# VasylVaskivskyi/microaligner

Measured on AMD Instinct MI355X. Metric: Mpix/s optical-flow reg+warp, 16k×16k float32 tile, 1/2/4/8 GPU, higher is better.
Workload: dtype f32

## Files before the change

### include/microaligner_hip.h

```cpp
#ifndef MICROALIGNER_HIP_H
#define MICROALIGNER_HIP_H

#include <stddef.h>
#include <stdint.h>

#ifdef __cplusplus
extern "C" {
#endif

typedef struct ma_ctx ma_ctx;

enum ma_dtype { MA_U8 = 0, MA_U16 = 1, MA_F32 = 2 };

enum ma_status {
    MA_OK = 0,
    MA_EINVAL = -1,
    MA_ENOMEM = -2,
    MA_EHIP = -3,
    MA_ENODEV = -4
};

enum ma_farneback_flags {
    MA_FB_MULADD_FUSED = 1
};

enum ma_dog_flags {
    MA_DOG_FUSED_BLUR = 1,
    MA_DOG_FUSED_SCALE = 2,
    MA_DOG_REPORT_ASYNC = 4
};

const char* ma_version(void);
const char* ma_last_error(void);
int ma_device_count(int* count);
int ma_ctx_create(int device, ma_ctx** out);
void ma_ctx_destroy(ma_ctx* ctx);
int ma_sync(ma_ctx* ctx);
int ma_ctx_set_workspace_limit(ma_ctx* ctx, size_t bytes);
void* ma_ctx_stream(ma_ctx* ctx);
int ma_ctx_trim(ma_ctx* ctx);
int ma_ctx_transfer_stats(ma_ctx* ctx, unsigned long long* h2d_bytes, unsigned long long* d2h_bytes, int reset);

enum ma_option { MA_OPT_COMPANION_STREAM = 1, MA_OPT_WORKSPACE_LIMIT = 2, MA_OPT_WARP_BAND_BYTES = 3 };
int ma_ctx_set_option(ma_ctx* ctx, int option, long long value);
int ma_ctx_get_option(ma_ctx* ctx, int option, long long* value);

enum ma_engine { MA_ENGINE_COMPUTE = 0, MA_ENGINE_H2D = 1, MA_ENGINE_D2H = 2 };
int ma_engine_memcpy_h2d(ma_ctx* ctx, int engine, void* dst, const void* src_host, size_t bytes);
int ma_engine_memcpy_d2h(ma_ctx* ctx, int engine, void* dst_host, const void* src, size_t bytes);
int ma_engine_record(ma_ctx* ctx, int engine, void* ev);
int ma_engine_wait(ma_ctx* ctx, int engine, void* ev);
int ma_engine_sync(ma_ctx* ctx, int engine);
int ma_host_parallel_copy(void* dst, const void* src, size_t bytes);
int ma_host_stream_copy(void* dst, const void* src, size_t bytes);
int ma_event_sync(ma_ctx* ctx, void* ev);

int ma_device_info(int device, char* name, size_t name_len, char* pci_bus_id, size_t pci_len, size_t* mem_free,
                   size_t* mem_total, int* compute_units);
int ma_clock_probe(ma_ctx* ctx, double milliseconds, double* sustained_ghz);

int ma_malloc(ma_ctx* ctx, size_t bytes, void** dptr);
int ma_free(ma_ctx* ctx, void* dptr);
int ma_memcpy_h2d(ma_ctx* ctx, void* dst, const void* src_host, size_t bytes);
int ma_memcpy_d2h(ma_ctx* ctx, void* dst_host, const void* src, size_t bytes);
int ma_memcpy_d2d(ma_ctx* ctx, void* dst, const void* src, size_t bytes);
int ma_memcpy_d2h_async(ma_ctx* ctx, void* dst_host, const void* src, size_t bytes);
int ma_host_alloc(size_t bytes, void** hptr);
int ma_host_free(void* hptr);
// ... 150 lines not shown
```

### microaligner_amd/_lib.py

```python
import ctypes as C
import os

_HERE = os.path.dirname(os.path.abspath(__file__))
LIB_PATH = os.environ.get("MICROALIGNER_HIP_LIB") or os.path.join(_HERE, "libmicroaligner_hip.so")

MA_U8, MA_U16, MA_F32 = 0, 1, 2
MA_OK, MA_EINVAL, MA_ENOMEM, MA_EHIP, MA_ENODEV = 0, -1, -2, -3, -4
MA_FB_MULADD_FUSED = 1
MA_KNN_AUTO, MA_KNN_EXACT, MA_KNN_FILTERED, MA_KNN_FILTERED_F32 = 0, 1, 2, 3
MA_DOG_FUSED_BLUR, MA_DOG_FUSED_SCALE, MA_DOG_REPORT_ASYNC = 1, 2, 4
MA_FLOW_CELL_REPLICAS = 8
MA_OPT_COMPANION_STREAM, MA_OPT_WORKSPACE_LIMIT, MA_OPT_WARP_BAND_BYTES = 1, 2, 3
MA_ENGINE_COMPUTE, MA_ENGINE_H2D, MA_ENGINE_D2H = 0, 1, 2

KERNEL_IDS = {"polyexp_m0": 0, "blur_v": 1, "blur_h_solve": 2, "warp": 3, "merge": 4, "pyr_down": 5,
              "pyr_up": 6, "dog": 7, "nmi": 8, "other": 9, "fb_level_img": 10, "fb_polyexp_plain": 11,
              "fb_flow_resize": 12, "fb_update_matrices": 13}

_vp, _i, _sz, _d, _f = C.c_void_p, C.c_int, C.c_size_t, C.c_double, C.c_float

SIGNATURES = {
    "ma_version": (C.c_char_p, []),
    "ma_last_error": (C.c_char_p, []),
    "ma_device_count": (_i, [C.POINTER(_i)]),
    "ma_ctx_create": (_i, [_i, C.POINTER(_vp)]),
    "ma_ctx_destroy": (None, [_vp]),
    "ma_sync": (_i, [_vp]),
    "ma_ctx_set_workspace_limit": (_i, [_vp, _sz]),
    "ma_ctx_stream": (_vp, [_vp]),
    "ma_malloc": (_i, [_vp, _sz, C.POINTER(_vp)]),
    "ma_free": (_i, [_vp, _vp]),
    "ma_memcpy_h2d": (_i, [_vp, _vp, _vp, _sz]),
    "ma_memcpy_d2h": (_i, [_vp, _vp, _vp, _sz]),
    "ma_memcpy_d2d": (_i, [_vp, _vp, _vp, _sz]),
    "ma_memcpy_d2h_async": (_i, [_vp, _vp, _vp, _sz]),
# ... 71 lines not shown
                              C.POINTER(MaFeatureRoundResult)]),
    "ma_ctx_trim": (_i, [_vp]),
    "ma_ctx_transfer_stats": (_i, [_vp, C.POINTER(C.c_ulonglong), C.POINTER(C.c_ulonglong), _i]),
    "ma_params_default": (None, [C.POINTER(MaParams)]),
    "ma_optflow_register": (_i, [_vp, _vp, _vp, _i, _i, _i, C.POINTER(MaParams), _vp, C.POINTER(MaLevelReport), _i,
                                 C.POINTER(_i)]),
    "ma_host_np_mean": (_i, [C.POINTER(_d), C.c_long, C.POINTER(_d)]),
    "ma_fast_keypoints": (_i, [_vp, _vp, _i, _i, _i, _i, _i, _vp, C.POINTER(_i)]),
    "ma_cut_tiles_u8": (_i, [_vp, _vp, _i, _i, _i, _i, _i, _i, _vp]),
    "ma_device_info": (_i, [_i, C.c_char_p, _sz, C.c_char_p, _sz, C.POINTER(_sz), C.POINTER(_sz), C.POINTER(_i)]),
    "ma_clock_probe": (_i, [_vp, _d, C.POINTER(_d)]),
    "ma_ctx_set_option": (_i, [_vp, _i, C.c_longlong]),
    "ma_ctx_get_option": (_i, [_vp, _i, C.POINTER(C.c_longlong)]),
    "ma_engine_memcpy_h2d": (_i, [_vp, _i, _vp, _vp, _sz]),
    "ma_engine_memcpy_d2h": (_i, [_vp, _i, _vp, _vp, _sz]),
    "ma_engine_record": (_i, [_vp, _i, _vp]),
    "ma_engine_wait": (_i, [_vp, _i, _vp]),
    "ma_engine_sync": (_i, [_vp, _i]),
    "ma_event_sync": (_i, [_vp, _vp]),
    "ma_host_parallel_copy": (_i, [_vp, _vp, _sz]),
    "ma_host_stream_copy": (_i, [_vp, _vp, _sz]),
    "ma_warp_pages_plan": (_i, [_i, _i, _i, _i, _i, _sz, C.POINTER(_i), C.POINTER(_i)]),
    "ma_convert_f32": (_i, [_vp, _vp, _i, _sz, _vp]),
})

QC_SIGNATURES = {
    "ma_qc_nmi_grid": (_i, [_vp, _vp, _vp, _vp, _i, _i, _i, _i, C.POINTER(_d), C.POINTER(_d), C.POINTER(_d), C.POINTER(_d)]),
    "ma_qc_flow_grid": (_i, [_vp, _vp, _i, _i, _i, _i, C.POINTER(_d), C.POINTER(C.c_longlong), C.POINTER(C.c_longlong),
                             C.POINTER(_d), C.POINTER(_d)]),
}

MA_INTER_NEAREST, MA_INTER_LINEAR, MA_INTER_CUBIC, MA_INTER_LANCZOS4 = 0, 1, 2, 4
INTERP_SIGNATURES = {
    "ma_remap_interp": (_i, [_vp, _vp, _i, _i, _i, _i, _vp, _i, _i, _vp, _i]),
    "ma_warp_tiled_interp": (_i, [_vp, _vp, _i, _i, _i, _vp, _i, _i, _vp, _i]),
    "ma_warp_pages_host_interp": (_i, [_vp, C.POINTER(_vp), C.POINTER(_vp), _i, _i, _i, _i, _vp, _i, _i, _i]),
}

COMPOSE_SIGNATURES = {
    "ma_warp_affine_flow": (_i, [_vp, _vp, _i, _i, _i, _i, _i, _vp, _i, _i, C.POINTER(_d), _vp, _i]),
    "ma_warp_affine_flow_pages_host": (_i, [_vp, C.POINTER(_vp), C.POINTER(_vp), _i, _i, _i, _i, _i, _i, _vp, _i, _i,
                                            C.POINTER(_d), _i]),
}

FLOWCOMPOSE_SIGNATURES = {
    "ma_compose_flows": (_i, [_vp, _vp, _vp, _i, _i, _vp]),
# ... 38 lines not shown
```

### microaligner_amd/csrc/farneback.hip

```cpp
#include "ma_internal.h"

#include <algorithm>
#include <cmath>
#include <cfloat>
#include <type_traits>

namespace {

struct FbGeom {
    MaTiling t;
    int pitch;
    int tile0;
    size_t plane;
    int margin;
};

struct PolyConsts {
    float g0, g1, xg1, xxg1;
    double ig11, ig03, ig33, ig55;
};

enum { PL_R0 = 0, PL_R1 = 5, PL_M = 10, PL_V = 15, PL_COUNT = 20 };

__device__ __forceinline__ float* plane_ptr(float* ws, const FbGeom& g, int wl, int pl)
// ... 204 lines not shown
                for (int k = 0; k < 5; k++)
                    __builtin_amdgcn_raw_buffer_store_b32(__float_as_uint(R[k]), wrsrc, pix4,
                                                          ((img == 0 ? PL_R0 : PL_R1) + k) * plane4, ST_NT);
            }
            if (img == 0) {
#pragma unroll
                for (int k = 0; k < 5; k++) r0v[rr][k] = R[k];
            } else if (ok) {
                const bool inside = x < Pw - 1 && y < Ph - 1;
                float Mv[5];
                update_matrices_px(r0v[rr], R[0], R[1], R[2], R[3], R[4], inside, 0.f, 0.f, x, y, Pw, Ph, Mv);
#pragma unroll
                for (int k = 0; k < 5; k++)
                    __builtin_amdgcn_raw_buffer_store_b32(__float_as_uint(Mv[k]), wrsrc, pix4, (PL_M + k) * plane4, ST_NT);
            }
        }
        __syncthreads();
    }
}

constexpr int BV_WAVES = 6, BH_WAVES = 4;
template <int R, int NW, bool FUSED>
__global__ __launch_bounds__(64 * NW, BV_WAVES) void fb_blur_v(FbGeom g, int m, const float* __restrict__ taps,
                                                     float* __restrict__ ws, int nplanes, int reach)
{
    extern __shared__ float lds[];
    const int lane = threadIdx.x & 63;
    const int w = __builtin_amdgcn_readfirstlane(threadIdx.x >> 6);
    const int Ph = g.t.Ph, Pw = g.t.Pw;
    const int nbx = (Pw + 63) / 64, nby = (Ph + NW * R - 1) / (NW * R);
    const int nslots = (int)(((nplanes + 7) / 8) * 8);
    const int item = d_xcd_work_item(blockIdx.x, nbx * nby * nslots);
    const int by = item % nby, bx = (item / nby) % nbx;
    const int bz = d_xcd_unit(item / (nby * nbx), nplanes);
    if (bz >= nplanes) return;
    const int wl = bz / 5, ch = bz - wl * 5;
    const float* src = plane_ptr(ws, g, wl, PL_M + ch);
    float* dst = plane_ptr(ws, g, wl, PL_V + ch);
    int oy, ox, ey, ex;
    window_origin(g.t, g.tile0 + wl, oy, ox);
    window_extent(g, oy, ox, ey, ex);
    const FbRect need = needed_rect_v(g.t, oy, ox, reach, m);
    const int x0 = (need.x0 & ~(NEED_XALIGN - 1)) + bx * 64, y0 = need.y0 + by * (NW * R);
    if (x0 >= min(ex, need.x1) || y0 >= min(ey, need.y1)) return;

    constexpr int G = 2;
    const int rows = NW * R + 2 * m + 2 * G;
    const int xc = min(x0 + lane, Pw - 1);
    const bool xin = xc < ex;
    {
        constexpr int SB = 42;
        const unsigned xo = (unsigned)xc * 4u;
        const __amdgpu_buffer_rsrc_t rsrc = __builtin_amdgcn_make_buffer_rsrc(const_cast<float*>(src), 0,
                                                                               (int)(g.plane * sizeof(float)), 0x00020000);
        for (int j0 = w; j0 < rows; j0 += NW * SB) {
            float v[SB];
#pragma unroll
            for (int k = 0; k < SB; k++) {
// ... 103 lines not shown
        }
        if (y0 + w * R < yend) {
            int jb = jbase + w * R;
            if (jb >= C) jb -= C;
            float acc[R];
            d_sym_fir_ring_pk<R, FUSED>(lds + lane, jb, C, m, taps, acc);
            if (x >= need.x0 && x < need.x1) {
#pragma unroll
                for (int r = 0; r < R; r++) {
                    const int y = y0 + w * R + r;
                    if (y < need.y1) __builtin_amdgcn_raw_buffer_store_b32(__float_as_uint(acc[r]), drsrc, x * 4, y * g.pitch * 4, 0);
                }
            }
        }
        jbase += CH;
        if (jbase >= C) jbase -= C;
        __syncthreads();
    }
}

template <int R, int NW, bool FUSED, int Q, bool LAST, int ROWS>
__global__ __launch_bounds__(64 * NW, BH_WAVES) void fb_blur_h_solve(FbGeom g, int m, const float* __restrict__ taps,
                                                           float* __restrict__ ws, float* __restrict__ flow_out,
                                                           int nwin, int reach)
{
    extern __shared__ float lds[];
    static_assert(ROWS == 64 || ROWS == 32, "a wave covers 64 rows, or 32 rows twice");
    constexpr int HALVES = 64 / ROWS;
    constexpr int TXW = NW * R * HALVES;
    constexpr int NT = 64 * NW;
    const int tid = threadIdx.x;
    const int lane = tid & 63;
    const int row = lane & (ROWS - 1);
    const int hcol = (lane / ROWS) * (NW * R);
    const int w = __builtin_amdgcn_readfirstlane(tid >> 6);
    const int Ph = g.t.Ph, Pw = g.t.Pw;
    const int nbx = (Pw + TXW - 1) / TXW, nby = (Ph + ROWS - 1) / ROWS;
    const int nslots = (int)(((nwin + 7) / 8) * 8);
    const int item = d_xcd_work_item(blockIdx.x, nbx * nby * nslots);
    const int bx = item % nbx, by = (item / nbx) % nby;
    const int wl = d_xcd_unit(item / (nbx * nby), nwin);
    if (wl >= nwin) return;
    int oy, ox, ey, ex;
    window_origin(g.t, g.tile0 + wl, oy, ox);
    window_extent(g, oy, ox, ey, ex);
    const FbRect need = needed_rect_h(g.t, oy, ox, reach);
    const int x0 = (need.x0 & ~(NEED_XALIGN - 1)) + bx * TXW, y0 = need.y0 + by * ROWS;
    const int xend = min(ex, need.x1), yend = min(ey, need.y1);
    if (x0 >= xend || y0 >= yend) return;
    constexpr int G = 2;
    const int cols = TXW + 2 * m + 2 * G;
    const int lp = cols | 1;

    constexpr int RW = ROWS / NW;
    float v[RW][Q];
    const int plane4 = (int)(g.plane * sizeof(float));
    const __amdgpu_buffer_rsrc_t wrsrc = __builtin_amdgcn_make_buffer_rsrc(plane_ptr(ws, g, wl, 0), 0, PL_COUNT * plane4, 0x00020000);
    int xo[Q];
#pragma unroll
    for (int q = 0; q < Q; q++) {
        const int xi = d_clamp(x0 - m - G + lane + 64 * q, 0, Pw - 1);
        xo[q] = xi >= ex ? (int)0x80000000 : xi * 4;
    }
    auto issue = [&](int ch) {
#pragma unroll
// ... 482 lines not shown
    const size_t lds_t = (size_t)BH_ROWS * (BH_TXW + 1) * 2 * sizeof(float);
    if (lds_t > lds_h) lds_h = lds_t;
    p.fast = m >= 1 && lds_v <= LDS_MAX && lds_h <= LDS_MAX && colsh <= 320;
    g.margin = p.fast ? (iters - 1) * m + 3 : (1 << 28);
    p.px = 0;
    p.px_v.assign(iters, 0.0);
    p.px_h.assign(iters, 0.0);
    for (int wl = 0; wl < nwin; wl++) {
        int oy = 0, ox = 0;
        if (g.t.T > 0) { int ty = (g.tile0 + wl) / g.t.ntx, tx = (g.tile0 + wl) % g.t.ntx; oy = ty * g.t.T - g.t.ov; ox = tx * g.t.T - g.t.ov; }
        const int vy = std::min(Ph, g.t.H - oy), vx = std::min(Pw, g.t.W - ox);
        const int ey = std::min(Ph, vy + std::min(g.margin, Ph)), ex = std::min(Pw, vx + std::min(g.margin, Pw));
        p.px += (double)ey * ex;
        for (int it = 0; it < iters; it++) {
            const int reach = p.fast ? (iters - 1 - it) * m : (1 << 28) / 2;
            const FbRect rh = needed_rect_h(g.t, oy, ox, reach), rv = needed_rect_v(g.t, oy, ox, reach, m);
            p.px_h[it] += (double)std::max(0, std::min(ey, rh.y1) - rh.y0) * std::max(0, std::min(ex, rh.x1) - rh.x0);
            p.px_v[it] += (double)std::max(0, std::min(ey, rv.y1) - rv.y0) * std::max(0, std::min(ex, rv.x1) - rv.x0);
        }
    }
    return p;
}

template <bool FUSED>
void run_iterations(ma_ctx* ctx, const FbGeom& g, const FbPlan& p, int nwin, int m, const float* taps, int iters,
                    float* flow_out)
{
    float* ws = (float*)ctx->ws;
    const int Ph = g.t.Ph, Pw = g.t.Pw;
    const size_t lds_v = (size_t)(BV_NW * BV_R + 2 * m + 4) * 64 * sizeof(float);
    const int colsh = BH_TXW + 2 * m + 4;
    size_t lds_h = (size_t)BH_ROWS * (colsh | 1) * sizeof(float);
    const size_t lds_t = (size_t)BH_ROWS * (BH_TXW + 1) * 2 * sizeof(float);
    if (lds_t > lds_h) lds_h = lds_t;
    const bool fast = p.fast;
    for (int it = 0; it < iters; it++) {
        const int last = it == iters - 1;
        const int reach = (iters - 1 - it) * m;
        if (fast) {
            {
                MaProfScope ps(ctx, MA_K_BLUR_V, p.px_v[it]);
                const size_t lds_vs = (size_t)(BVS_NW * BV_R + 2 * m + 4 + 3 * (BV_R / 2) + 1) * 64 * sizeof(float);
                if (m % (BV_R / 2) == 0 && lds_vs <= LDS_MAX) {
                    const long long items = (long long)((Pw + 63) / 64) * nwin * 5;
                    hipLaunchKernelGGL((fb_blur_v_stream<BV_R, BVS_NW, FUSED>), dim3((unsigned)items), dim3(64 * BVS_NW),
                                       lds_vs, ctx->stream, g, m, taps, ws, nwin * 5, reach);
                } else {
                    const long long items = (long long)((Pw + 63) / 64) * ((Ph + BV_NW * BV_R - 1) / (BV_NW * BV_R)) * ma_xcd_slots(nwin * 5);
                    hipLaunchKernelGGL((fb_blur_v<BV_R, BV_NW, FUSED>), dim3(ma_xcd_grid(items)), dim3(64 * BV_NW), lds_v,
                                       ctx->stream, g, m, taps, ws, nwin * 5, reach);
                }
            }
            {
                MaProfScope ps(ctx, MA_K_BLUR_H_SOLVE, p.px_h[it]);
                const long long items = (long long)((Pw + BH_TXW - 1) / BH_TXW) * ((Ph + BH_ROWS - 1) / BH_ROWS) * ma_xcd_slots(nwin);
#define MA_BLUR_H(QQ)                                                                                               \
    do {                                                                                                            \
        if (last) hipLaunchKernelGGL((fb_blur_h_solve<BH_R, BH_NW, FUSED, QQ, true, BH_ROWS>), dim3(ma_xcd_grid(items)),     \
                                     dim3(64 * BH_NW), lds_h, ctx->stream, g, m, taps, ws, flow_out, nwin, reach);  \
        else hipLaunchKernelGGL((fb_blur_h_solve<BH_R, BH_NW, FUSED, QQ, false, BH_ROWS>), dim3(ma_xcd_grid(items)),         \
                                dim3(64 * BH_NW), lds_h, ctx->stream, g, m, taps, ws, flow_out, nwin, reach);       \
    } while (0)
                if (colsh <= 192) MA_BLUR_H(3);
                else if (colsh <= 256) MA_BLUR_H(4);
                else MA_BLUR_H(5);
#undef MA_BLUR_H
            }
        } else {
            {
                MaProfScope ps(ctx, MA_K_BLUR_V, p.px);
                dim3 grid((Pw + 255) / 256, Ph, nwin * 5);
                hipLaunchKernelGGL((fb_blur_v_simple<FUSED>), grid, dim3(256), 0, ctx->stream, g, m, taps, ws);
            }
            {
                MaProfScope ps(ctx, MA_K_BLUR_H_SOLVE, p.px);
                dim3 grid((Pw + 255) / 256, Ph, nwin);
                hipLaunchKernelGGL((fb_blur_h_solve_simple<FUSED>), grid, dim3(256), 0, ctx->stream, g, m, taps, ws,
                                   last, flow_out);
            }
        }
    }
}

template <typename T, bool FUSED>
int run_batch(ma_ctx* ctx, const T* prev, const T* next, FbGeom g, int nwin, const PolyConsts& pc, int m,
              const float* taps, int iters, float* flow_out)
{
    float* ws = (float*)ctx->ws;
    const FbPlan p = plan_batch(g, nwin, m, iters);
    {
        MaProfScope ps(ctx, MA_K_POLYEXP_M0, p.px);
        dim3 grid((g.t.Pw + K1_TX - 1) / K1_TX, (g.t.Ph + K1_TY - 1) / K1_TY, nwin);
        hipLaunchKernelGGL((fb_polyexp_m0<T>), grid, dim3(K1_THREADS), 0, ctx->stream, prev, next, g, pc, ws);
    }
    run_iterations<FUSED>(ctx, g, p, nwin, m, taps, iters, flow_out);
    MA_HIP(hipGetLastError());
    return MA_OK;
}

int get_taps(ma_ctx* ctx, int winsize, const float** out)
{
    std::vector<float> k;
    make_window_taps(winsize, k);
    std::vector<float> t = ma_layout_taps(k);
    return ma_const_table(ctx, ((uint64_t)1 << 56) | (uint64_t)winsize, t.data(), t.size(), out);
}

int check_window(int Ph, int Pw)
{
    const size_t bytes = ma_fb_window_bytes(Ph, Pw);
    if (bytes <= MA_FB_WINDOW_MAX_BYTES) return MA_OK;
    ma_set_error("invalid argument: Farneback window of %d x %d px too large: its 20 planes take %zu bytes, the 32-bit "
                 "plane addressing allows %zu (5178 x 5178 is the largest square window)", Ph, Pw, bytes,
                 MA_FB_WINDOW_MAX_BYTES);
    return MA_EINVAL;
}

int farneback_impl(ma_ctx* ctx, const void* prev, const void* next, int dtype, int H, int W, int tile, int overlap,
// ... 136 lines not shown
                for (int img = 0; img < 2; img++) {
                    hipLaunchKernelGGL((fb_level_rows<T, FUSED>), dim3((2 * l.w + LV_THREADS - 1) / LV_THREADS,
                                       (unsigned)std::min(H, MA_GRID_Y_MAX)), dim3(LV_THREADS), 0, ctx->stream,
                                       img == 0 ? prev : next, H, W, l.w, sx, dk, l.ksize, tmp);
                    hipLaunchKernelGGL((fb_level_cols<FUSED>), dim3((l.w + 255) / 256, gy), dim3(256), 0, ctx->stream, tmp, H,
                                       W, l.w, l.h, sx, sy, area, dk, l.ksize, ws + (PL_V + img) * g.plane, g.pitch);
                }
            }
            MaProfScope ps(ctx, MA_K_FB_POLYEXP_PLAIN, 2 * px);
            hipLaunchKernelGGL(fb_polyexp_plain, dim3((l.w + 255) / 256, gy, 2), dim3(256), 0, ctx->stream, g, pc, ws);
        }
        if (k == top) {
            MA_HIP(hipMemsetAsync(flow_out, 0, (size_t)l.w * l.h * 2 * sizeof(float), ctx->stream));
        } else {
            const FbLevel& c = L[k + 1];
            MaProfScope ps(ctx, MA_K_FB_FLOW_RESIZE, px);
            hipLaunchKernelGGL((fb_flow_resize<FUSED>), dim3((l.w + 255) / 256, gy), dim3(256), 0, ctx->stream, flow_lv,
                               c.w, c.h, rs_scale(l.w, c.w), rs_scale(l.h, c.h), flow_out, l.w, l.h);
        }
        {
            MaProfScope ps(ctx, MA_K_FB_UPDATE_MATRICES, px);
            hipLaunchKernelGGL(fb_update_matrices, dim3((l.w + 255) / 256, gy), dim3(256), 0, ctx->stream, g, flow_out, ws);
        }
        run_iterations<FUSED>(ctx, g, p, 1, m, taps, iters, k == 0 ? flow_out : flow_lv);
        MA_HIP(hipGetLastError());
    }
    return MA_OK;
}

int farneback_levels_impl(ma_ctx* ctx, const void* prev, const void* next, int dtype, int H, int W, int levels,
                          double pyr_scale, int winsize, int iterations, int poly_n, double poly_sigma, int flags,
                          float* flow_out)
{
    MA_REQUIRE(levels >= 0, "levels must be >= 0");
    MA_REQUIRE(pyr_scale == 0.5, "only pyr_scale == 0.5 is supported");
    if (levels == 0)
        return farneback_impl(ctx, prev, next, dtype, H, W, 0, 0, winsize, iterations, poly_n, poly_sigma, flags, flow_out,
                              nullptr, nullptr, nullptr);
    MA_REQUIRE(ctx && prev && next && flow_out, "NULL argument");
    MA_REQUIRE(dtype == MA_U8 || dtype == MA_U16 || dtype == MA_F32, "dtype must be u8/u16/f32");
    MA_REQUIRE(H > 0 && W > 0, "image must be non-empty");
    MA_REQUIRE(winsize >= 1, "winsize must be >= 1");
    MA_REQUIRE(iterations >= 1, "iterations must be >= 1");
    MA_REQUIRE(poly_n == 1, "only poly_n == 1 is supported (the value microaligner passes)");
    const std::vector<FbLevel> L = level_table(H, W, levels);
    if (L.size() == 1)
        return farneback_impl(ctx, prev, next, dtype, H, W, 0, 0, winsize, iterations, poly_n, poly_sigma, flags, flow_out,
// ... 8 lines not shown
    const float* taps = nullptr;
    MA_TRY(get_taps(ctx, winsize, &taps));
    MA_TRY(ma_ws_reserve(ctx, lw.total * sizeof(float)));
    const bool fused = (flags & MA_FB_MULADD_FUSED) != 0;
    const int m = winsize / 2;
#define RUN(TYPE)                                                                                                      \
    (fused ? run_levels<TYPE, true>(ctx, (const TYPE*)prev, (const TYPE*)next, H, W, L, lw.flow_off, pc, m, taps,      \
                                    iterations, flow_out)                                                              \
           : run_levels<TYPE, false>(ctx, (const TYPE*)prev, (const TYPE*)next, H, W, L, lw.flow_off, pc, m, taps,     \
                                     iterations, flow_out))
    if (dtype == MA_U8) return RUN(uint8_t);
    if (dtype == MA_U16) return RUN(uint16_t);
    return RUN(float);
#undef RUN
}

}

size_t ma_fb_window_bytes(int Ph, int Pw)
{
    return (size_t)Ph * ma_align_up((size_t)Pw, 64) * PL_COUNT * sizeof(float);
}

extern "C" {

int ma_farneback_tiled(ma_ctx* ctx, const void* prev, const void* next, int dtype, int H, int W, int tile,
                       int overlap, int winsize, int iterations, int poly_n, double poly_sigma, int flags,
                       float* flow_out)
{
    return farneback_impl(ctx, prev, next, dtype, H, W, tile, overlap, winsize, iterations, poly_n, poly_sigma,
                          flags, flow_out, nullptr, nullptr, nullptr);
}

int ma_farneback_levels(ma_ctx* ctx, const void* prev, const void* next, int dtype, int H, int W, int levels,
                        double pyr_scale, int winsize, int iterations, int poly_n, double poly_sigma, int flags,
                        float* flow_out)
{
    return farneback_levels_impl(ctx, prev, next, dtype, H, W, levels, pyr_scale, winsize, iterations, poly_n, poly_sigma,
                                 flags, flow_out);
}

int ma_farneback_debug(ma_ctx* ctx, const void* prev, const void* next, int dtype, int H, int W, int winsize,
                       int iterations, double poly_sigma, int flags, float* flow_out, float* R0_planar,
                       float* R1_planar, float* M0_planar)
{
    return farneback_impl(ctx, prev, next, dtype, H, W, 0, 0, winsize, iterations, 1, poly_sigma, flags, flow_out,
                          R0_planar, R1_planar, M0_planar);
// ... 4 lines not shown
```

### microaligner_amd/csrc/ma_api.hip

```cpp
#include "ma_internal.h"

#include <chrono>
#include "ma_src_hash.h"

#include <condition_variable>
#include <pthread.h>
#include <sched.h>
#include <unistd.h>
#include <cstring>
#include <map>
#include <mutex>
#include <thread>

static thread_local std::string g_last_error;

void ma_set_error(const char* fmt, ...)
{
    char buf[1024];
    va_list ap;
    va_start(ap, fmt);
    vsnprintf(buf, sizeof(buf), fmt, ap);
    va_end(ap);
    g_last_error = buf;
}
// ... 45 lines not shown
    hipError_t e = hipStreamCreateWithFlags(&ctx->stream, hipStreamNonBlocking);
    if (e != hipSuccess) {
        delete ctx;
        ma_set_error("hipStreamCreate failed: %s", hipGetErrorString(e));
        return MA_EHIP;
    }
    *out = ctx;
    return MA_OK;
}

void ma_ctx_destroy(ma_ctx* ctx)
{
    if (!ctx) return;
    (void)hipSetDevice(ctx->device);
    (void)hipStreamSynchronize(ctx->stream);
    if (ctx->side) { ma_ctx_destroy(ctx->side); ctx->side = nullptr; }
    for (auto e : ctx->sync_events) (void)hipEventDestroy(e);
    for (auto& r : ctx->pending) { (void)hipEventDestroy(r.a); (void)hipEventDestroy(r.b); }
    for (auto e : ctx->free_events) (void)hipEventDestroy(e);
    for (auto& kv : ctx->pool_free) (void)hipFree(kv.second);
    for (auto& kv : ctx->pool_live) (void)hipFree(kv.first);
    if (ctx->ws) (void)hipFree(ctx->ws);
    if (ctx->dconst) (void)hipFree(ctx->dconst);
    if (ctx->pinned) (void)hipHostFree(ctx->pinned);
    if (ctx->dog_sticky_buf) (void)hipFree(ctx->dog_sticky_buf);
    if (ctx->round_flags) (void)hipHostFree(ctx->round_flags);
    for (int e = 1; e < 3; e++)
        if (ctx->engine[e]) { (void)hipStreamSynchronize(ctx->engine[e]); (void)hipStreamDestroy(ctx->engine[e]); }
    ma_stage_rings_destroy(ctx);
    (void)hipStreamDestroy(ctx->stream);
    delete ctx;
}

int ma_sync(ma_ctx* ctx)
{
    MA_REQUIRE(ctx, "ctx is NULL");
    MA_HIP(hipStreamSynchronize(ctx->stream));
    return MA_OK;
}

int ma_ctx_set_workspace_limit(ma_ctx* ctx, size_t bytes)
{
    MA_REQUIRE(ctx, "ctx is NULL");
    MA_REQUIRE(bytes >= ((size_t)1 << 20), "workspace limit must be >= 1 MiB");
    ctx->ws_limit = bytes;
    return MA_OK;
}

int ma_ctx_set_option(ma_ctx* ctx, int option, long long value)
{
    MA_REQUIRE(ctx, "ctx is NULL");
    switch (option) {
    case MA_OPT_COMPANION_STREAM:
        ctx->companion = value != 0;
        return MA_OK;
    case MA_OPT_WORKSPACE_LIMIT:
        MA_REQUIRE(value > 0, "workspace limit must be positive");
        return ma_ctx_set_workspace_limit(ctx, (size_t)value);
    case MA_OPT_WARP_BAND_BYTES:
        MA_REQUIRE(value > 0, "band size must be positive");
        ctx->warp_band_bytes = (size_t)value;
        return MA_OK;
    default:
        ma_set_error("invalid argument: unknown option %d", option);
        return MA_EINVAL;
    }
}

int ma_ctx_get_option(ma_ctx* ctx, int option, long long* value)
{
    MA_REQUIRE(ctx && value, "NULL argument");
    switch (option) {
    case MA_OPT_COMPANION_STREAM: *value = ctx->companion ? 1 : 0; return MA_OK;
    case MA_OPT_WORKSPACE_LIMIT: *value = (long long)ctx->ws_limit; return MA_OK;
    case MA_OPT_WARP_BAND_BYTES: *value = (long long)ctx->warp_band_bytes; return MA_OK;
    default:
        ma_set_error("invalid argument: unknown option %d", option);
        return MA_EINVAL;
    }
}

void* ma_ctx_stream(ma_ctx* ctx) { return ctx ? (void*)ctx->stream : nullptr; }

int ma_ctx_trim(ma_ctx* ctx)
{
    MA_REQUIRE(ctx, "ctx is NULL");
    MA_HIP(hipSetDevice(ctx->device));
    MA_HIP(hipStreamSynchronize(ctx->stream));
    for (auto& kv : ctx->pool_free) (void)hipFree(kv.second);
    ctx->pool_free.clear();
    if (ctx->side) {
        ma_ctx* sd = ctx->side;
        MA_HIP(hipStreamSynchronize(sd->stream));
        for (auto& kv : sd->pool_free) (void)hipFree(kv.second);
        sd->pool_free.clear();
        if (sd->ws) { (void)hipFree(sd->ws); sd->ws = nullptr; sd->ws_bytes = 0; }
    }
    return MA_OK;
// ... 905 lines not shown
```

### microaligner_amd/csrc/ma_internal.h

```cpp
#pragma once
#include <hip/hip_runtime.h>

#include <atomic>
#include <cstdarg>
#include <cstdint>
#include <cstdio>
#include <map>
#include <mutex>
#include <string>
#include <unordered_map>
#include <utility>
#include <functional>
#include <vector>

#include "../../include/microaligner_hip.h"

void ma_set_error(const char* fmt, ...);
struct MaStageRing;

#define MA_HIP(expr)                                                                          \
    do {                                                                                      \
        hipError_t _e = (expr);                                                               \
        if (_e != hipSuccess) {                                                               \
            ma_set_error("%s failed: %s (%s:%d)", #expr, hipGetErrorString(_e), __FILE__, __LINE__); \
// ... 21 lines not shown
    void* ws = nullptr;
    size_t ws_bytes = 0;
    size_t ws_limit = (size_t)48 << 30;
    void* pinned = nullptr;
    size_t pinned_bytes = 0;
    void* dconst = nullptr;
    size_t dconst_bytes = 0;
    bool profile = false;
    struct Rec { hipEvent_t a, b; int id; };
    std::vector<Rec> pending;
    std::vector<hipEvent_t> free_events;
    double prof_ms[MA_K_COUNT] = {0};
    long long prof_n[MA_K_COUNT] = {0};
    double prof_px[MA_K_COUNT] = {0};
    std::multimap<size_t, void*> pool_free;
    std::unordered_map<void*, size_t> pool_live;
    std::atomic<unsigned long long> h2d_bytes{0}, d2h_bytes{0};
    hipStream_t engine[3] = {nullptr, nullptr, nullptr};
    std::mutex mu;
    MaStageRing* stage[3][2] = {{nullptr, nullptr}, {nullptr, nullptr}, {nullptr, nullptr}};
    std::mutex stage_mu[3][2];
    bool companion = true;
    size_t warp_band_bytes = (size_t)32 << 20;
    int* dog_sticky = nullptr;
    int* dog_sticky_buf = nullptr;
    int* round_flags = nullptr;
    ma_ctx* side = nullptr;
    std::vector<hipEvent_t> sync_events;
};
ma_ctx* ma_ctx_side(ma_ctx* ctx);
void ma_stage_rings_destroy(ma_ctx* ctx);
constexpr int MA_GRID_Y_MAX = 65535;
hipStream_t ma_engine_stream(ma_ctx* ctx, int engine);
typedef std::function<int(int)> MaPieceFn;
int ma_engine_h2d_pieces(ma_ctx* ctx, int engine, void* dst, const void* src_host, size_t bytes, const size_t* cuts, int ncuts,
                         const MaPieceFn& enqueued, bool wait = true);
int ma_engine_d2h_pieces(ma_ctx* ctx, int engine, void* dst_host, const void* src, size_t bytes, const size_t* cuts, int ncuts,
                         const MaPieceFn& before);
struct MaPagePlan {
    size_t in_bytes, out_bytes;
    size_t out_row_bytes;
    std::vector<size_t> cuts_src;
    std::vector<size_t> cuts_out;
};
typedef std::function<int(const void* din, void* dout, int y0, int y1)> MaBandFn;
int ma_warp_pages_run(ma_ctx* ctx, const void* const* pages_host, void* const* out_host, int n_pages, const MaPagePlan& plan,
// ... 241 lines not shown
    if ((threadIdx.x & 63) == 0) { s_lo[threadIdx.x >> 6] = lo; s_hi[threadIdx.x >> 6] = hi; }
    __syncthreads();
    if (threadIdx.x == 0) {
        for (int k = 1; k < nw; k++) { lo = fminf(lo, s_lo[k]); hi = fmaxf(hi, s_hi[k]); }
        part[0] = lo; part[1] = hi;
    }
}
int ma_launch_minmax_final(ma_ctx* ctx, const float* part, int nparts, float* out2);

__device__ __forceinline__ int d_xcd_work_item(int b, int n_items)
{
    const int per = (n_items + 7) >> 3;
    return (b & 7) * per + (b >> 3);
}
static inline unsigned ma_xcd_grid(long long n_items) { return (unsigned)(((n_items + 7) / 8) * 8); }

__device__ __forceinline__ int d_xcd_unit(int slot, int n_units)
{
    const int per = (n_units + 7) >> 3;
    return (slot % per) * 8 + slot / per;
}
static inline long long ma_xcd_slots(long long n_units) { return ((n_units + 7) / 8) * 8; }

struct MaTiling {
    int H, W;
    int T, ov;
    int ntx, nty;
    int Ph, Pw;
};

static inline MaTiling ma_make_tiling(int H, int W, int tile, int overlap)
{
    MaTiling g;
    g.H = H; g.W = W;
    if (tile <= 0) {
        g.T = 0; g.ov = 0; g.ntx = g.nty = 1; g.Ph = H; g.Pw = W;
    } else {
        g.T = tile; g.ov = overlap;
        g.ntx = (W + tile - 1) / tile; g.nty = (H + tile - 1) / tile;
        g.Ph = g.Pw = tile + 2 * overlap;
    }
    return g;
}

constexpr size_t MA_FB_WINDOW_MAX_BYTES = (size_t)INT32_MAX;
size_t ma_fb_window_bytes(int Ph, int Pw);
// ... 1 lines not shown
```

### microaligner_amd/device.py

```python
import collections
import ctypes as C
import os
import threading
import weakref
import zlib

import numpy as np

from . import _lib as L

_DT = {np.dtype(np.uint8): L.MA_U8, np.dtype(np.uint16): L.MA_U16, np.dtype(np.float32): L.MA_F32}


def _dt(dtype):
    dtype = np.dtype(dtype)
    if dtype not in _DT:
        raise ValueError(f"unsupported image dtype {dtype}: the HIP path handles uint8, uint16 and float32")
    return _DT[dtype]


INTERPOLATIONS = {"nearest": L.MA_INTER_NEAREST, "linear": L.MA_INTER_LINEAR, "cubic": L.MA_INTER_CUBIC,
                  "lanczos4": L.MA_INTER_LANCZOS4}


# ... 336 lines not shown
                self._host_pool.setdefault(bucket, []).append(ptr)
                return
        self.lib.ma_host_free(ptr)

    def sync(self):
        L.check(self.lib.ma_sync(self.handle))

    def set_option(self, option, value):
        L.check(self.lib.ma_ctx_set_option(self.handle, int(option), int(value)))

    def get_option(self, option):
        v = C.c_longlong()
        L.check(self.lib.ma_ctx_get_option(self.handle, int(option), C.byref(v)))
        return v.value

    @property
    def companion_stream(self):
        return bool(self.get_option(L.MA_OPT_COMPANION_STREAM))

    @companion_stream.setter
    def companion_stream(self, on):
        self.set_option(L.MA_OPT_COMPANION_STREAM, 1 if on else 0)

    def engine_upload(self, dst, arr, engine=L.MA_ENGINE_H2D):
        if arr.nbytes != dst.nbytes or not arr.flags.c_contiguous:
            raise ValueError("engine_upload needs a C-contiguous host array of the device array's size")
        _warn_if_staged_on_a_full_node(arr)
        L.check(self.lib.ma_engine_memcpy_h2d(self.handle, int(engine), dst.ptr, arr.ctypes.data, arr.nbytes))

    def engine_download(self, src, out, engine=L.MA_ENGINE_D2H):
        if out.nbytes != src.nbytes or not out.flags.c_contiguous:
            raise ValueError("engine_download needs a C-contiguous host array of the device array's size")
        _warn_if_staged_on_a_full_node(out)
        L.check(self.lib.ma_engine_memcpy_d2h(self.handle, int(engine), out.ctypes.data, src.ptr, out.nbytes))

    def engine_record(self, engine, ev):
        L.check(self.lib.ma_engine_record(self.handle, int(engine), ev))

    def engine_wait(self, engine, ev):
        L.check(self.lib.ma_engine_wait(self.handle, int(engine), ev))

    def engine_sync(self, engine):
        L.check(self.lib.ma_engine_sync(self.handle, int(engine)))

    def event_sync(self, ev):
        L.check(self.lib.ma_event_sync(self.handle, ev))
# ... 55 lines not shown

    def record(self, ev):
        L.check(self.lib.ma_event_record(self.handle, ev))

    def elapsed_ms(self, a, b):
        ms = C.c_float()
        L.check(self.lib.ma_event_elapsed_ms(self.handle, a, b, C.byref(ms)))
        return ms.value

    def profile(self, on=True):
        L.check(self.lib.ma_profile_enable(self.handle, int(on)))

    def profile_reset(self):
        L.check(self.lib.ma_profile_reset(self.handle))

    def profile_get(self):
        out = {}
        for name, kid in L.KERNEL_IDS.items():
            ms, n, px = C.c_double(), C.c_longlong(), C.c_double()
            L.check(self.lib.ma_profile_get(self.handle, kid, C.byref(ms), C.byref(n), C.byref(px)))
            out[name] = {"ms": ms.value, "launches": n.value, "px": px.value}
        return out

    def farneback(self, prev, nxt, winsize, iterations, tile=0, overlap=0, poly_n=1, poly_sigma=1.7, fused=False, levels=0):
        if prev.shape != nxt.shape or prev.ndim != 2:
            raise ValueError("prev/next must be 2-D arrays of the same shape")
        if levels > 0 and tile > 0:
            raise ValueError("levels > 0 runs on the whole image: tile must be 0")
        if prev.dtype != nxt.dtype:
            prev, nxt = self.to_f32(prev), self.to_f32(nxt)
        H, W = prev.shape
        flow = self.empty((H, W, 2), np.float32)
        if levels > 0:
            self._run(self.lib.ma_farneback_levels, prev.ptr, nxt.ptr, _dt(prev.dtype), H, W, int(levels), 0.5,
                      int(winsize), int(iterations), int(poly_n), float(poly_sigma),
                      L.MA_FB_MULADD_FUSED if fused else 0, flow.ptr)
            return flow
        self._run(self.lib.ma_farneback_tiled, prev.ptr, nxt.ptr, _dt(prev.dtype), H, W, int(tile),
                                            int(overlap), int(winsize), int(iterations), int(poly_n),
                                            float(poly_sigma), L.MA_FB_MULADD_FUSED if fused else 0, flow.ptr)
        return flow

    def farneback_debug(self, prev, nxt, winsize, iterations, poly_sigma=1.7, fused=False):
        H, W = prev.shape
        flow = self.empty((H, W, 2), np.float32)
        r0, r1, m0 = (self.empty((5, H, W), np.float32) for _ in range(3))
        self._run(self.lib.ma_farneback_debug, prev.ptr, nxt.ptr, _dt(prev.dtype), H, W, int(winsize),
                                            int(iterations), float(poly_sigma),
                                            L.MA_FB_MULADD_FUSED if fused else 0, flow.ptr, r0.ptr, r1.ptr, m0.ptr)
        return flow, r0, r1, m0

    def optflow_register(self, ref, mov, num_pyr_lvl=4, num_iterations=3, tile_size=1000, overlap=100,
                         use_full_res_img=False, use_dog=False, fb_flags=0, dog_flags=0):
        if ref.shape != mov.shape or ref.dtype != mov.dtype or ref.ndim != 2:
            raise ValueError("ref/mov must be 2-D images of equal shape and dtype")
# ... 651 lines not shown
```

Baseline: 3574.

## Balance Farneback blur work across XCDs with planned band groups and order

```diff
diff --git a/include/microaligner_hip.h b/include/microaligner_hip.h
--- a/include/microaligner_hip.h
+++ b/include/microaligner_hip.h
@@ -41,9 +41,11 @@
 int ma_ctx_trim(ma_ctx* ctx);
 int ma_ctx_transfer_stats(ma_ctx* ctx, unsigned long long* h2d_bytes, unsigned long long* d2h_bytes, int reset);
 
-enum ma_option { MA_OPT_COMPANION_STREAM = 1, MA_OPT_WORKSPACE_LIMIT = 2, MA_OPT_WARP_BAND_BYTES = 3 };
+enum ma_option { MA_OPT_COMPANION_STREAM = 1, MA_OPT_WORKSPACE_LIMIT = 2, MA_OPT_WARP_BAND_BYTES = 3, MA_OPT_FB_XCD_BANDS = 4 };
 int ma_ctx_set_option(ma_ctx* ctx, int option, long long value);
 int ma_ctx_get_option(ma_ctx* ctx, int option, long long* value);
+int ma_xcd_plan(int n_parents, const int* len, const int* cross, int n_blocks, int block_px, int* blocks_per_unit, int* order,
+                int capacity, int* n_units);
 
 enum ma_engine { MA_ENGINE_COMPUTE = 0, MA_ENGINE_H2D = 1, MA_ENGINE_D2H = 2 };
 int ma_engine_memcpy_h2d(ma_ctx* ctx, int engine, void* dst, const void* src_host, size_t bytes);
diff --git a/microaligner_amd/_lib.py b/microaligner_amd/_lib.py
--- a/microaligner_amd/_lib.py
+++ b/microaligner_amd/_lib.py
@@ -10,7 +10,7 @@
 MA_KNN_AUTO, MA_KNN_EXACT, MA_KNN_FILTERED, MA_KNN_FILTERED_F32 = 0, 1, 2, 3
 MA_DOG_FUSED_BLUR, MA_DOG_FUSED_SCALE, MA_DOG_REPORT_ASYNC = 1, 2, 4
 MA_FLOW_CELL_REPLICAS = 8
-MA_OPT_COMPANION_STREAM, MA_OPT_WORKSPACE_LIMIT, MA_OPT_WARP_BAND_BYTES = 1, 2, 3
+MA_OPT_COMPANION_STREAM, MA_OPT_WORKSPACE_LIMIT, MA_OPT_WARP_BAND_BYTES, MA_OPT_FB_XCD_BANDS = 1, 2, 3, 4
 MA_ENGINE_COMPUTE, MA_ENGINE_H2D, MA_ENGINE_D2H = 0, 1, 2
 
 KERNEL_IDS = {"polyexp_m0": 0, "blur_v": 1, "blur_h_solve": 2, "warp": 3, "merge": 4, "pyr_down": 5,
@@ -128,6 +128,7 @@
     "ma_host_stream_copy": (_i, [_vp, _vp, _sz]),
     "ma_warp_pages_plan": (_i, [_i, _i, _i, _i, _i, _sz, C.POINTER(_i), C.POINTER(_i)]),
     "ma_convert_f32": (_i, [_vp, _vp, _i, _sz, _vp]),
+    "ma_xcd_plan": (_i, [_i, C.POINTER(_i), C.POINTER(_i), _i, _i, C.POINTER(_i), C.POINTER(_i), _i, C.POINTER(_i)]),
 })
 
 QC_SIGNATURES = {
diff --git a/microaligner_amd/csrc/farneback.hip b/microaligner_amd/csrc/farneback.hip
--- a/microaligner_amd/csrc/farneback.hip
+++ b/microaligner_amd/csrc/farneback.hip
@@ -250,18 +250,23 @@
 constexpr int BV_WAVES = 6, BH_WAVES = 4;
 template <int R, int NW, bool FUSED>
 __global__ __launch_bounds__(64 * NW, BV_WAVES) void fb_blur_v(FbGeom g, int m, const float* __restrict__ taps,
-                                                     float* __restrict__ ws, int nplanes, int reach)
+                                                     float* __restrict__ ws, int nplanes, int reach, int kb,
+                                                     const int* __restrict__ order)
 {
     extern __shared__ float lds[];
     const int lane = threadIdx.x & 63;
     const int w = __builtin_amdgcn_readfirstlane(threadIdx.x >> 6);
     const int Ph = g.t.Ph, Pw = g.t.Pw;
     const int nbx = (Pw + 63) / 64, nby = (Ph + NW * R - 1) / (NW * R);
-    const int nslots = (int)(((nplanes + 7) / 8) * 8);
-    const int item = d_xcd_work_item(blockIdx.x, nbx * nby * nslots);
-    const int by = item % nby, bx = (item / nby) % nbx;
-    const int bz = d_xcd_unit(item / (nby * nbx), nplanes);
-    if (bz >= nplanes) return;
+    const int nsg = (nbx + kb - 1) / kb, nunits = nplanes * nsg;
+    const int nslots = (int)(((nunits + 7) / 8) * 8);
+    const int item = d_xcd_work_item(blockIdx.x, nby * kb * nslots);
+    const int by = item % nby;
+    const int ui = d_xcd_unit(item / (nby * kb), nunits);
+    if (ui >= nunits) return;
+    const int unit = order ? order[ui] : ui;
+    const int bz = unit / nsg, bx = (unit - bz * nsg) * kb + (item / nby) % kb;
+    if (bx >= nbx) return;
     const int wl = bz / 5, ch = bz - wl * 5;
     const float* src = plane_ptr(ws, g, wl, PL_M + ch);
     float* dst = plane_ptr(ws, g, wl, PL_V + ch);
@@ -411,7 +416,7 @@
 template <int R, int NW, bool FUSED, int Q, bool LAST, int ROWS>
 __global__ __launch_bounds__(64 * NW, BH_WAVES) void fb_blur_h_solve(FbGeom g, int m, const float* __restrict__ taps,
                                                            float* __restrict__ ws, float* __restrict__ flow_out,
-                                                           int nwin, int reach)
+                                                           int nwin, int reach, int kb, const int* __restrict__ order)
 {
     extern __shared__ float lds[];
     static_assert(ROWS == 64 || ROWS == 32, "a wave covers 64 rows, or 32 rows twice");
@@ -425,11 +430,15 @@
     const int w = __builtin_amdgcn_readfirstlane(tid >> 6);
     const int Ph = g.t.Ph, Pw = g.t.Pw;
     const int nbx = (Pw + TXW - 1) / TXW, nby = (Ph + ROWS - 1) / ROWS;
-    const int nslots = (int)(((nwin + 7) / 8) * 8);
-    const int item = d_xcd_work_item(blockIdx.x, nbx * nby * nslots);
-    const int bx = item % nbx, by = (item / nbx) % nby;
-    const int wl = d_xcd_unit(item / (nbx * nby), nwin);
-    if (wl >= nwin) return;
+    const int nbg = (nby + kb - 1) / kb, nunits = nwin * nbg;
+    const int nslots = (int)(((nunits + 7) / 8) * 8);
+    const int item = d_xcd_work_item(blockIdx.x, nbx * kb * nslots);
+    const int bx = item % nbx;
+    const int ui = d_xcd_unit(item / (nbx * kb), nunits);
+    if (ui >= nunits) return;
+    const int unit = order ? order[ui] : ui;
+    const int wl = unit / nbg, by = (unit - wl * nbg) * kb + (item / nbx) % kb;
+    if (by >= nby) return;
     int oy, ox, ey, ex;
     window_origin(g.t, g.tile0 + wl, oy, ox);
     window_extent(g, oy, ox, ey, ex);
@@ -958,8 +967,46 @@
     return p;
 }
 
+struct FbList { int kb; const int* order; };
+int fb_work_list(ma_ctx* ctx, const FbGeom& g, int nwin, int m, int reach, bool vertical, int nb, int bsize, FbList* out)
+{
+    if (!ctx->fb_xcd_bands) { out->kb = nb; out->order = nullptr; return MA_OK; }
+    const std::vector<int> key = {vertical ? 1 : 0, g.t.H, g.t.W, g.t.T, g.t.ov, g.tile0, nwin, m, reach, g.margin, nb, bsize};
+    auto it = ctx->fb_lists.find(key);
+    if (it == ctx->fb_lists.end()) {
+        const int per = vertical ? 5 : 1;
+        std::vector<int> len((size_t)nwin * per), cross((size_t)nwin * per), order;
+        for (int wl = 0; wl < nwin; wl++) {
+            int oy = 0, ox = 0;
+            if (g.t.T > 0) { const int ty = (g.tile0 + wl) / g.t.ntx, tx = (g.tile0 + wl) % g.t.ntx; oy = ty * g.t.T - g.t.ov; ox = tx * g.t.T - g.t.ov; }
+            const int vy = std::min(g.t.Ph, g.t.H - oy), vx = std::min(g.t.Pw, g.t.W - ox);
+            const int ey = std::min(g.t.Ph, vy + std::min(g.margin, g.t.Ph)), ex = std::min(g.t.Pw, vx + std::min(g.margin, g.t.Pw));
+            const FbRect r = vertical ? needed_rect_v(g.t, oy, ox, reach, m) : needed_rect_h(g.t, oy, ox, reach);
+            const int rows = std::max(0, std::min(ey, r.y1) - r.y0);
+            for (int k = 0; k < per; k++) {
+                len[(size_t)wl * per + k] = vertical ? std::max(0, std::min(ex, r.x1) - (r.x0 & ~(NEED_XALIGN - 1))) : rows;
+                cross[(size_t)wl * per + k] = vertical ? rows : std::max(0, std::min(ex, r.x1) - r.x0);
+            }
+        }
+        const int kb = ma_xcd_plan_units(nwin * per, len.data(), cross.data(), nb, bsize, &order);
+        if (ctx->fb_lists.size() >= 256) {
+            MA_HIP(hipStreamSynchronize(ctx->stream));
+            for (auto& kv : ctx->fb_lists) (void)hipFree(kv.second.second);
+            ctx->fb_lists.clear();
+        }
+        int* d = nullptr;
+        MA_HIP(hipMalloc((void**)&d, order.size() * sizeof(int)));
+        hipError_t e = hipMemcpy(d, order.data(), order.size() * sizeof(int), hipMemcpyHostToDevice);
+        if (e != hipSuccess) { (void)hipFree(d); MA_HIP(e); }
+        it = ctx->fb_lists.emplace(key, std::make_pair(kb, d)).first;
+    }
+    out->kb = it->second.first;
+    out->order = it->second.second;
+    return MA_OK;
+}
+
 template <bool FUSED>
-void run_iterations(ma_ctx* ctx, const FbGeom& g, const FbPlan& p, int nwin, int m, const float* taps, int iters,
+int run_iterations(ma_ctx* ctx, const FbGeom& g, const FbPlan& p, int nwin, int m, const float* taps, int iters,
                     float* flow_out)
 {
     float* ws = (float*)ctx->ws;
@@ -974,28 +1021,36 @@
         const int last = it == iters - 1;
         const int reach = (iters - 1 - it) * m;
         if (fast) {
+            const size_t lds_vs = (size_t)(BVS_NW * BV_R + 2 * m + 4 + 3 * (BV_R / 2) + 1) * 64 * sizeof(float);
+            const bool stream_v = m % (BV_R / 2) == 0 && lds_vs <= LDS_MAX;
+            FbList lv = {0, nullptr}, lh = {0, nullptr};
+            if (!stream_v) MA_TRY(fb_work_list(ctx, g, nwin, m, reach, true, (Pw + 63) / 64, 64, &lv));
+            MA_TRY(fb_work_list(ctx, g, nwin, m, reach, false, (Ph + BH_ROWS - 1) / BH_ROWS, BH_ROWS, &lh));
             {
                 MaProfScope ps(ctx, MA_K_BLUR_V, p.px_v[it]);
-                const size_t lds_vs = (size_t)(BVS_NW * BV_R + 2 * m + 4 + 3 * (BV_R / 2) + 1) * 64 * sizeof(float);
-                if (m % (BV_R / 2) == 0 && lds_vs <= LDS_MAX) {
+                if (stream_v) {
                     const long long items = (long long)((Pw + 63) / 64) * nwin * 5;
                     hipLaunchKernelGGL((fb_blur_v_stream<BV_R, BVS_NW, FUSED>), dim3((unsigned)items), dim3(64 * BVS_NW),
                                        lds_vs, ctx->stream, g, m, taps, ws, nwin * 5, reach);
                 } else {
-                    const long long items = (long long)((Pw + 63) / 64) * ((Ph + BV_NW * BV_R - 1) / (BV_NW * BV_R)) * ma_xcd_slots(nwin * 5);
+                    const int nbx = (Pw + 63) / 64;
+                    const long long items = (long long)lv.kb * ((Ph + BV_NW * BV_R - 1) / (BV_NW * BV_R)) *
+                                            ma_xcd_slots((long long)nwin * 5 * ((nbx + lv.kb - 1) / lv.kb));
                     hipLaunchKernelGGL((fb_blur_v<BV_R, BV_NW, FUSED>), dim3(ma_xcd_grid(items)), dim3(64 * BV_NW), lds_v,
-                                       ctx->stream, g, m, taps, ws, nwin * 5, reach);
+                                       ctx->stream, g, m, taps, ws, nwin * 5, reach, lv.kb, lv.order);
                 }
             }
             {
                 MaProfScope ps(ctx, MA_K_BLUR_H_SOLVE, p.px_h[it]);
-                const long long items = (long long)((Pw + BH_TXW - 1) / BH_TXW) * ((Ph + BH_ROWS - 1) / BH_ROWS) * ma_xcd_slots(nwin);
+                const int nby = (Ph + BH_ROWS - 1) / BH_ROWS;
+                const long long items = (long long)((Pw + BH_TXW - 1) / BH_TXW) * lh.kb *
+                                        ma_xcd_slots((long long)nwin * ((nby + lh.kb - 1) / lh.kb));
 #define MA_BLUR_H(QQ)                                                                                               \
     do {                                                                                                            \
         if (last) hipLaunchKernelGGL((fb_blur_h_solve<BH_R, BH_NW, FUSED, QQ, true, BH_ROWS>), dim3(ma_xcd_grid(items)),     \
-                                     dim3(64 * BH_NW), lds_h, ctx->stream, g, m, taps, ws, flow_out, nwin, reach);  \
+                                     dim3(64 * BH_NW), lds_h, ctx->stream, g, m, taps, ws, flow_out, nwin, reach, lh.kb, lh.order);  \
         else hipLaunchKernelGGL((fb_blur_h_solve<BH_R, BH_NW, FUSED, QQ, false, BH_ROWS>), dim3(ma_xcd_grid(items)),         \
-                                dim3(64 * BH_NW), lds_h, ctx->stream, g, m, taps, ws, flow_out, nwin, reach);       \
+                                dim3(64 * BH_NW), lds_h, ctx->stream, g, m, taps, ws, flow_out, nwin, reach, lh.kb, lh.order);       \
     } while (0)
                 if (colsh <= 192) MA_BLUR_H(3);
                 else if (colsh <= 256) MA_BLUR_H(4);
@@ -1016,6 +1071,7 @@
             }
         }
     }
+    return MA_OK;
 }
 
 template <typename T, bool FUSED>
@@ -1029,7 +1085,7 @@
         dim3 grid((g.t.Pw + K1_TX - 1) / K1_TX, (g.t.Ph + K1_TY - 1) / K1_TY, nwin);
         hipLaunchKernelGGL((fb_polyexp_m0<T>), grid, dim3(K1_THREADS), 0, ctx->stream, prev, next, g, pc, ws);
     }
-    run_iterations<FUSED>(ctx, g, p, nwin, m, taps, iters, flow_out);
+    MA_TRY(run_iterations<FUSED>(ctx, g, p, nwin, m, taps, iters, flow_out));
     MA_HIP(hipGetLastError());
     return MA_OK;
 }
@@ -1212,7 +1268,7 @@
             MaProfScope ps(ctx, MA_K_FB_UPDATE_MATRICES, px);
             hipLaunchKernelGGL(fb_update_matrices, dim3((l.w + 255) / 256, gy), dim3(256), 0, ctx->stream, g, flow_out, ws);
         }
-        run_iterations<FUSED>(ctx, g, p, 1, m, taps, iters, k == 0 ? flow_out : flow_lv);
+        MA_TRY(run_iterations<FUSED>(ctx, g, p, 1, m, taps, iters, k == 0 ? flow_out : flow_lv));
         MA_HIP(hipGetLastError());
     }
     return MA_OK;
@@ -1267,7 +1323,56 @@
     return (size_t)Ph * ma_align_up((size_t)Pw, 64) * PL_COUNT * sizeof(float);
 }
 
+int ma_xcd_plan_units(int np, const int* len, const int* cross, int nb, int bsize, std::vector<int>* order)
+{
+    std::vector<long long> wt;
+    std::vector<int> idx, best;
+    int best_k = nb;
+    long long best_max = -1;
+    for (int ng = 1, prev_k = 0; ng <= nb; ng++) {
+        const int k = (nb + ng - 1) / ng;
+        if (k == prev_k) continue;
+        prev_k = k;
+        const int nbg = (nb + k - 1) / k;
+        const size_t nu = (size_t)np * nbg;
+        wt.resize(nu);
+        long long total = 0;
+        for (int p = 0; p < np; p++)
+            for (int gi = 0; gi < nbg; gi++) {
+                const long long px = std::min<long long>(std::max<long long>((long long)len[p] - (long long)gi * k * bsize, 0),
+                                                         (long long)k * bsize);
+                total += wt[(size_t)p * nbg + gi] = px * cross[p];
+            }
+        idx.resize(nu);
+        for (size_t u = 0; u < nu; u++) idx[u] = (int)u;
+        std::stable_sort(idx.begin(), idx.end(), [&](int a, int b) { return wt[a] > wt[b]; });
+        long long load[8] = {0, 0, 0, 0, 0, 0, 0, 0}, mx = 0;
+        for (size_t i = 0; i < nu; i++) load[i & 7] += wt[idx[i]];
+        for (int x = 0; x < 8; x++) mx = std::max(mx, load[x]);
+        const bool balanced = (double)mx * 8 <= (double)total * (1.0 + MA_XCD_TOLERANCE);
+        if (best_max < 0 || mx < best_max || balanced) { best_max = mx; best_k = k; best.swap(idx); }
+        if (balanced) break;
+    }
+    order->swap(best);
+    return best_k;
+}
+
 extern "C" {
+
+int ma_xcd_plan(int n_parents, const int* len, const int* cross, int n_blocks, int block_px, int* blocks_per_unit, int* order,
+                int capacity, int* n_units)
+{
+    MA_REQUIRE(len && cross && blocks_per_unit && order && n_units, "NULL argument");
+    MA_REQUIRE(n_parents >= 1 && n_blocks >= 1 && block_px >= 1, "counts must be positive");
+    MA_REQUIRE((long long)n_parents * n_blocks <= capacity, "order holds fewer than n_parents * n_blocks ints");
+    for (int p = 0; p < n_parents; p++)
+        MA_REQUIRE(len[p] >= 0 && len[p] <= (long long)n_blocks * block_px && cross[p] >= 0, "len / cross out of range");
+    std::vector<int> o;
+    *blocks_per_unit = ma_xcd_plan_units(n_parents, len, cross, n_blocks, block_px, &o);
+    *n_units = (int)o.size();
+    std::copy(o.begin(), o.end(), order);
+    return MA_OK;
+}
 
 int ma_farneback_tiled(ma_ctx* ctx, const void* prev, const void* next, int dtype, int H, int W, int tile,
                        int overlap, int winsize, int iterations, int poly_n, double poly_sigma, int flags,
diff --git a/microaligner_amd/csrc/ma_api.hip b/microaligner_amd/csrc/ma_api.hip
--- a/microaligner_amd/csrc/ma_api.hip
+++ b/microaligner_amd/csrc/ma_api.hip
@@ -91,6 +91,7 @@
     for (auto& kv : ctx->pool_live) (void)hipFree(kv.first);
     if (ctx->ws) (void)hipFree(ctx->ws);
     if (ctx->dconst) (void)hipFree(ctx->dconst);
+    for (auto& kv : ctx->fb_lists) (void)hipFree(kv.second.second);
     if (ctx->pinned) (void)hipHostFree(ctx->pinned);
     if (ctx->dog_sticky_buf) (void)hipFree(ctx->dog_sticky_buf);
     if (ctx->round_flags) (void)hipHostFree(ctx->round_flags);
@@ -130,6 +131,9 @@
         MA_REQUIRE(value > 0, "band size must be positive");
         ctx->warp_band_bytes = (size_t)value;
         return MA_OK;
+    case MA_OPT_FB_XCD_BANDS:
+        ctx->fb_xcd_bands = value != 0;
+        return MA_OK;
     default:
         ma_set_error("invalid argument: unknown option %d", option);
         return MA_EINVAL;
@@ -143,6 +147,7 @@
     case MA_OPT_COMPANION_STREAM: *value = ctx->companion ? 1 : 0; return MA_OK;
     case MA_OPT_WORKSPACE_LIMIT: *value = (long long)ctx->ws_limit; return MA_OK;
     case MA_OPT_WARP_BAND_BYTES: *value = (long long)ctx->warp_band_bytes; return MA_OK;
+    case MA_OPT_FB_XCD_BANDS: *value = ctx->fb_xcd_bands ? 1 : 0; return MA_OK;
     default:
         ma_set_error("invalid argument: unknown option %d", option);
         return MA_EINVAL;
diff --git a/microaligner_amd/csrc/ma_internal.h b/microaligner_amd/csrc/ma_internal.h
--- a/microaligner_amd/csrc/ma_internal.h
+++ b/microaligner_amd/csrc/ma_internal.h
@@ -67,6 +67,8 @@
     std::mutex stage_mu[3][2];
     bool companion = true;
     size_t warp_band_bytes = (size_t)32 << 20;
+    bool fb_xcd_bands = true;
+    std::map<std::vector<int>, std::pair<int, int*>> fb_lists;
     int* dog_sticky = nullptr;
     int* dog_sticky_buf = nullptr;
     int* round_flags = nullptr;
@@ -354,6 +356,9 @@
 }
 static inline long long ma_xcd_slots(long long n_units) { return ((n_units + 7) / 8) * 8; }
 
+constexpr double MA_XCD_TOLERANCE = 0.03;
+int ma_xcd_plan_units(int np, const int* len, const int* cross, int nb, int bsize, std::vector<int>* order);
+
 struct MaTiling {
     int H, W;
     int T, ov;
diff --git a/microaligner_amd/device.py b/microaligner_amd/device.py
--- a/microaligner_amd/device.py
+++ b/microaligner_amd/device.py
@@ -382,6 +382,14 @@
     def companion_stream(self, on):
         self.set_option(L.MA_OPT_COMPANION_STREAM, 1 if on else 0)
 
+    @property
+    def fb_xcd_bands(self):
+        return bool(self.get_option(L.MA_OPT_FB_XCD_BANDS))
+
+    @fb_xcd_bands.setter
+    def fb_xcd_bands(self, on):
+        self.set_option(L.MA_OPT_FB_XCD_BANDS, 1 if on else 0)
+
     def engine_upload(self, dst, arr, engine=L.MA_ENGINE_H2D):
         if arr.nbytes != dst.nbytes or not arr.flags.c_contiguous:
             raise ValueError("engine_upload needs a C-contiguous host array of the device array's size")
@@ -483,7 +491,8 @@
             out[name] = {"ms": ms.value, "launches": n.value, "px": px.value}
         return out
 
-    def farneback(self, prev, nxt, winsize, iterations, tile=0, overlap=0, poly_n=1, poly_sigma=1.7, fused=False, levels=0):
+    def farneback(self, prev, nxt, winsize, iterations, tile=0, overlap=0, poly_n=1, poly_sigma=1.7, fused=False, levels=0,
+                  out=None):
         if prev.shape != nxt.shape or prev.ndim != 2:
             raise ValueError("prev/next must be 2-D arrays of the same shape")
         if levels > 0 and tile > 0:
@@ -491,7 +500,9 @@
         if prev.dtype != nxt.dtype:
             prev, nxt = self.to_f32(prev), self.to_f32(nxt)
         H, W = prev.shape
-        flow = self.empty((H, W, 2), np.float32)
+        if out is not None and (out.shape != (H, W, 2) or out.dtype != np.float32):
+            raise ValueError("out must be an (H, W, 2) float32 array")
+        flow = out if out is not None else self.empty((H, W, 2), np.float32)
         if levels > 0:
             self._run(self.lib.ma_farneback_levels, prev.ptr, nxt.ptr, _dt(prev.dtype), H, W, int(levels), 0.5,
                       int(winsize), int(iterations), int(poly_n), float(poly_sigma),
```

After: 3606 (median of 6 runs). Within noise of the previous version (+0.9%).
